# zihang-student/Codes-of-IPD-SsN-AMG-method

Hardware: AMD Instinct MI355X
Metric: V-cycle throughput (DoF*cycles/sec), m=n=1024 OT grid (higher is better)
Workload: dtype f64

## Files before the change

codes_of_ipd_ssn_amg_method_amd/csrc/ipd_resident.h:

```cpp
#pragma once

#include "ipd_resident_proto.h"

static constexpr int RES_P3_LD = 1152;
static constexpr int RES_P4_LD = 2 * RES_P4_SEG + 64;

struct ResLevelDesc {
    int N, nf, S;
    const unsigned short* pci;
    const double* pva;
    const double* diag;
    const double* dinv;
    const double* Axi;
    const double* xx;
};
struct ResDesc {
    ResLevelDesc L1, L2;
    ResLevelDesc L3;
    ResCsr Pt2, P2;
    ResCsr Pt3, P3;
    ResCsr Pt4, P4;
    ResCsr A3;
    ResCsr A4;
    int three;
    const double* p3rows;
    const double* p3w;
    const double* p2rows;
    const double* p2w;
    int p2seg, p2ld;
    int N5;
    const double* p4rows;
    const double* p4w;
    int remote;
    ResTail tail;
    int xm, xm_nwf, xm_nwc;
    const unsigned long long* xm_fbits;
    const unsigned long long* xm_cbits;
    const double* xm_beta;
    const double* xm_rho;
    int localfirst;
    int wident;
    int Nt;
    int nu, isnsp, wcycle, anycycle, maxit;
    double retol;
    long long pcg_maxit;
    unsigned char* gran0;
    unsigned char* gran1;
    int presleep;
    int pollsleep;
    unsigned* tmo;
    long long* dbg;
    unsigned dbg_skip_seq;
};

template <int KE>
// ... 43 lines not shown
    double y[KE];
#pragma unroll
    for (int q = 0; q < KE / 2; ++q) {
        asm volatile("" : "+v"(c[q]));
        const unsigned lo = c[q] & 0xffffu, hi = c[q] >> 16;
        y[2 * q] = *reinterpret_cast<const double*>(smb + OFFB + lo);
        y[2 * q + 1] = *reinterpret_cast<const double*>(smb + OFFB + hi);
    }
    double s0 = a[0] * y[0], s1 = a[1] * y[1], s2 = a[2] * y[2], s3 = a[3] * y[3];
#pragma unroll
    for (int q = 4; q < KE; q += 4) {
        s0 = __builtin_fma(a[q], y[q], s0);
        s1 = __builtin_fma(a[q + 1], y[q + 1], s1);
        s2 = __builtin_fma(a[q + 2], y[q + 2], s2);
        s3 = __builtin_fma(a[q + 3], y[q + 3], s3);
    }
    return (s0 + s1) + (s2 + s3);
}

__device__ __forceinline__ double res_csr_rowdot(const ResCsr& M, int e0, int e1, int lane,
                                                 const double* sm, int off) {
    double s = 0.0;
    for (int t = e0 + lane; t < e1; t += 64 * 8) {
        int jj[8];
        double aa[8];
#pragma unroll
        for (int u = 0; u < 8; ++u) {
            const int tt = t + 64 * u;
            const int tc = tt < e1 ? tt : e0;
            jj[u] = M.ci[tc];
            aa[u] = M.va[tc];
        }
#pragma unroll
        for (int u = 0; u < 8; ++u) s += (t + 64 * u < e1) ? aa[u] * sm[off + jj[u]] : 0.0;
    }
    return wave_sum(s);
}

__device__ __forceinline__ double res_red8(const double* red) {
    double t = 0.0;
#pragma unroll
    for (int k = 0; k < RES_WAVES; ++k) t += red[k];
    return t;
}

__device__ __forceinline__ double res_red8_tree(const double* red) {
    static_assert(RES_WAVES == 8, "eight waves");
    double v[RES_WAVES];
#pragma unroll
    for (int k = 0; k < RES_WAVES; ++k) v[k] = red[k];
    return ((v[0] + v[1]) + (v[2] + v[3])) + ((v[4] + v[5]) + (v[6] + v[7]));
}

__device__ __forceinline__ void res_swap_halves32(double& a, double& b) {
    const auto lo = __builtin_amdgcn_permlane32_swap((unsigned)__double2loint(a), (unsigned)__double2loint(b), false, false);
    const auto hi = __builtin_amdgcn_permlane32_swap((unsigned)__double2hiint(a), (unsigned)__double2hiint(b), false, false);
    a = __hiloint2double((int)hi[0], (int)lo[0]);
    b = __hiloint2double((int)hi[1], (int)lo[1]);
}
__device__ __forceinline__ void res_swap_rows16(double& a, double& b) {
    const auto lo = __builtin_amdgcn_permlane16_swap((unsigned)__double2loint(a), (unsigned)__double2loint(b), false, false);
    const auto hi = __builtin_amdgcn_permlane16_swap((unsigned)__double2hiint(a), (unsigned)__double2hiint(b), false, false);
    a = __hiloint2double((int)hi[0], (int)lo[0]);
    b = __hiloint2double((int)hi[1], (int)lo[1]);
}
__device__ __forceinline__ void res_cs_rows(const double (&A)[RES_WAVES][2], double v0, double v1, double* part_out,
                                            int w, int lane) {
    static_assert(RES_WAVES == 8, "eight rows per block and workgroup");
    double p[RES_WAVES];
#pragma unroll
    for (int r = 0; r < RES_WAVES; ++r) p[r] = __builtin_fma(A[r][1], v1, A[r][0] * v0);
    double q[4];
#pragma unroll
    for (int k = 0; k < 4; ++k) {
        res_swap_halves32(p[k], p[k + 4]);
        q[k] = p[k] + p[k + 4];
    }
    double t[2];
#pragma unroll
    for (int k = 0; k < 2; ++k) {
        res_swap_rows16(q[k], q[k + 2]);
        t[k] = q[k] + q[k + 2];
    }
    const bool f = (lane & 8) != 0;
    const double keep = f ? t[1] : t[0], send = f ? t[0] : t[1];
    double u = keep + dpp_get<0x128, 0xf>(send);
    u = subwave_sum(u, 8);
    if ((lane & 7) == 0) part_out[8 * (lane >> 3) + w] = u;
}

enum res_class {
    RES_CL_HALF = 0,
    RES_CL_START = 1,
    RES_CL_RR = 2,
    RES_CL_RESTRICT = 3,
    RES_CL_LEVEL2 = 4,
    RES_CL_PROLONG = 5,
    RES_CL_TOP = 6,
    RES_NCLASS = 8
};

template <int KE1, int KE2, int KE3 = 0, bool POLY2 = false, bool DIAG = true, bool FULL = false>
__global__ __launch_bounds__(BT, 2) void k_resident(const ResDesc D, const double* __restrict__ bvec,
                                                    double* xg, double* out, int fixed_cycles) {
    static_assert(!POLY2 || (KE3 == 0 && KE1 == 16), "POLY2: three-level hierarchies in column slices (resident_takes_poly2)");
    static_assert(!FULL || POLY2, "FULL: the composed instantiation only (resident_takes_full)");
    static_assert(DIAG || KE1 == 16, "the production form exists for the column-slice kernels");
    constexpr int FG = 2 * BT / RES_WAVES;
    if constexpr (FULL) __builtin_assume(__builtin_amdgcn_workitem_id_x() < (unsigned)BT);
    constexpr bool THREE = KE3 > 0;
    constexpr bool POLY3 = KE3 == 1;
    constexpr int K3 = (THREE && !POLY3) ? KE3 : 2;
    extern __shared__ __attribute__((aligned(16))) char res_smem[];
    double* sm = reinterpret_cast<double*>(res_smem);
    const char* smb = res_smem;
    const int tid = threadIdx.x, w = tid >> 6, lane = tid & 63;
#define RES_REMOTE (FULL ? 0 : D.remote)
#define RES_WIDENT (FULL ? 1 : D.wident)
    const int b = blockIdx.x, G = FULL ? FG : gridDim.x - (RES_REMOTE ? 1 : 0);
    const int N1 = FULL ? 4 * BT : D.L1.N, N2 = FULL ? 2 * BT : D.L2.N, nf = FULL ? 2 * BT : D.L1.nf, nc = N1 - nf;
    const int Nt = FULL ? 1 : D.Nt;
    if (RES_REMOTE && b == G) {
        __shared__ PhaseLds tail_lds;
        __shared__ double tail_red[16];
        __shared__ double tail_part[48 + SOLVE_ML + 1];
        __shared__ int tail_stat[RES_WAVES];
        res_tail_workgroup(D.tail, res_smem, &tail_lds, tail_red, tail_part, tail_stat);
        return;
    }
    constexpr int oX = 0, oE1 = RES_NMAX, oE2 = 2 * RES_NMAX, oRR1 = 3 * RES_NMAX;
    constexpr int oR1 = 4 * RES_NMAX, oAX1 = 5 * RES_NMAX, oR2 = 6 * RES_NMAX, oRR2 = 7 * RES_NMAX;
    constexpr int oAX2 = 8 * RES_NMAX;
    constexpr int oRHO = 9 * RES_NMAX;
    constexpr int oBETA = oAX2 + RES_NMAX / 2;
    constexpr int oU = oRR2;
    constexpr int oR3 = 9 * RES_NMAX + RES_NMAX / 2, oE3 = oR3 + RES_TAIL_MAX, oP3 = oE3 + RES_TAIL_MAX;
    constexpr int oPART = oR3, oPART9 = oR3 + 2 * RES_WAVES * RES_WAVES;
    static_assert(2 * RES_WAVES * RES_WAVES + 2 * RES_WAVES <= 3 * RES_TAIL_MAX, "the totals fit the tail's slots");
    constexpr int oRED = oP3 + RES_TAIL_MAX;
    constexpr int oPUB = oRED + 2 * RES_WAVES;
    constexpr int oOWN = oPUB + 2 * RES_WAVES;
// ... 127 lines not shown
        rowp[12 * w + 2] = D.P2.rp[rF];
        rowp[12 * w + 3] = vF ? D.P2.rp[rF + 1] : D.P2.rp[rF];
        rowp[12 * w + 4] = D.P2.rp[rC];
        rowp[12 * w + 5] = vC ? D.P2.rp[rC + 1] : D.P2.rp[rC];
        const int rin = b + G * w;
        const ResCsr& Pin = D.tail.root == 4 ? D.Pt4 : D.Pt3;
        rowp[12 * w + 6] = (RES_REMOTE && rin < Nt) ? Pin.rp[rin] : 0;
        rowp[12 * w + 7] = (RES_REMOTE && rin < Nt) ? Pin.rp[rin + 1] : 0;
        rowp[12 * w + 8] = v3 ? D.Pt3.rp[r3] : 0;
        rowp[12 * w + 9] = v3 ? D.Pt3.rp[r3 + 1] : 0;
        rowp[12 * w + 10] = (THREE && v2) ? D.P3.rp[r2] : 0;
        rowp[12 * w + 11] = (THREE && v2) ? D.P3.rp[r2 + 1] : 0;
    }
#define dgF sm[oOWN + 0 * RES_WAVES + w]
#define dvF sm[oOWN + 1 * RES_WAVES + w]
#define bF sm[oOWN + 2 * RES_WAVES + w]
#define dgC sm[oOWN + 3 * RES_WAVES + w]
#define dvC sm[oOWN + 4 * RES_WAVES + w]
#define bC sm[oOWN + 5 * RES_WAVES + w]
#define dg2 sm[oOWN + 6 * RES_WAVES + w]
#define dv2 sm[oOWN + 7 * RES_WAVES + w]
#define dg3 sm[oOWN + 8 * RES_WAVES + w]
#define dv3 sm[oOWN + 9 * RES_WAVES + w]
    const bool nsp = FULL ? true : D.isnsp != 0;
    const double xx1 = nsp ? D.L1.xx[0] : 1.0, xx2 = nsp ? D.L2.xx[0] : 1.0;
    const double xx3 = (THREE && nsp) ? D.L3.xx[0] : 1.0;
    const double rxx1 = 1.0 / xx1, rxx2 = 1.0 / xx2, rxx3 = 1.0 / xx3;
    for (int j = tid; j < N1; j += BT) {
        sm[oX + j] = xg[j];
        sm[oE1 + j] = 0.0;
        sm[oAX1 + j] = D.L1.Axi[j];
    }
    for (int j = tid; j < N2; j += BT) {
        sm[oE2 + j] = 0.0;
        sm[oAX2 + j] = D.L2.Axi[j];
    }
    if (THREE)
        for (int j = tid; j < N3; j += BT) {
            sm[oE3L + j] = 0.0;
            sm[oAX3L + j] = D.L3.Axi[j];
        }
    const bool tail1 = FULL ? true : !THREE && Nt == 1 && N2 <= RES_NMAX / 2;
    constexpr int oP3C = oRR2 + RES_NMAX / 2;
    const bool lfirst = FULL ? true : D.localfirst && D.nu >= 1 && N2 <= RES_NMAX / 2 && nf <= RES_NMAX / 2;
    const bool lfirst2 = lfirst && !THREE;
    constexpr int oDV1 = oR2 + RES_NMAX / 2, oDV2 = oE2 + RES_NMAX / 2;
    if (lfirst) {
        for (int j = tid; j < nf; j += BT) sm[oDV1 + j] = D.L1.dinv[j];
        if (lfirst2)
            for (int j = tid; j < N2; j += BT) sm[oDV2 + j] = D.L2.dinv[j];
    }
    const bool xm = FULL ? true : !THREE && D.xm != 0 && nc == N2 && D.wident != 0;
    unsigned xbits = 0;
    if (xm) {
        unsigned long long wf[16], wc[16];
#pragma unroll
        for (int q = 0; q < 16; ++q) {
            wf[q] = D.xm_fbits[(size_t)rF * D.xm_nwf + (q < D.xm_nwf ? q : 0)];
            wc[q] = D.xm_cbits[(size_t)(rC - nf) * D.xm_nwc + (q < D.xm_nwc ? q : 0)];
        }
        unsigned lo = 0, hi = 0;
#pragma unroll
        for (int q = 0; q < 16; ++q) {
            lo |= (vF && q < D.xm_nwf) ? (unsigned)((wf[q] >> lane) & 1ull) << q : 0u;
            hi |= (vC && q < D.xm_nwc) ? (unsigned)((wc[q] >> lane) & 1ull) << q : 0u;
        }
        xbits = lo | (hi << 16);
        for (int j = tid; j < nf; j += BT) sm[oRHO + j] = D.xm_rho[j];
        for (int j = tid; j < nc; j += BT) sm[oBETA + j] = D.xm_beta[j];
    }
    double h33 = 0.0;
    if (tail1) {
        for (int j = tid; j < N2; j += BT) {
            double v = 0.0;
            if (POLY2) {
                v = D.p2rows[(size_t)N2 * D.p2ld + j];
            } else {
                for (int t = D.P3.rp[j]; t < D.P3.rp[j + 1]; ++t)
                    if (D.P3.ci[t] == 0) v = D.P3.va[t];
            }
            sm[oP3C + j] = v;
        }
        for (int t = D.A3.rp[0]; t < D.A3.rp[1]; ++t)
            if (D.A3.ci[t] == 0) h33 = D.A3.va[t];
    }
    if (tid == 0) *fail = 0;
    __syncthreads();

    const auto rs = __builtin_amdgcn_make_buffer_rsrc(D.gran0, 0, 2 * RES_GRAN_MAX * 16, 0x00020000);
    unsigned seq = 0;
    bool dead = false;
    const bool dbg = DIAG && D.dbg != nullptr && b == 0 && tid == 0;
#define RES_SKIPPED(sq) (DIAG && (sq) == D.dbg_skip_seq && b == G - 1)
    if (dbg) {
        dbg_acc[0] = dbg_acc[3] = dbg_acc[4] = dbg_acc[5] = dbg_acc[6] = dbg_acc[7] = dbg_acc[8] = 0;
        dbg_acc[1] = __builtin_amdgcn_s_memtime();
        dbg_acc[2] = __builtin_amdgcn_s_memrealtime();
        if constexpr (KE1 == 16)
            for (int k = 0; k < 2 * RES_NCLASS; ++k) cls_acc[k] = 0u;
    }
    auto cls_begin = [&](int c) __attribute__((always_inline)) {
        if constexpr (KE1 == 16) {
            if (dbg) __hip_atomic_fetch_sub(cls_acc + c, (unsigned)__builtin_amdgcn_s_memtime(), __ATOMIC_RELAXED, __HIP_MEMORY_SCOPE_WORKGROUP);
        }
    };
    auto cls_end = [&](int c) __attribute__((always_inline)) {
// ... 106 lines not shown
    (void)csFed; (void)csBuf; (void)eFo; (void)eCo;
    bool topfed = false;
    (void)topfed;
    auto cs_both_rows = [&](int off) __attribute__((always_inline)) {
        const double f0 = tid < nc ? sm[off + nf + tid] : 0.0, f1 = tid + BT < nc ? sm[off + nf + tid + BT] : 0.0;
        const double g0 = tid < nf ? sm[off + tid] : 0.0, g1 = tid + BT < nf ? sm[off + tid + BT] : 0.0;
        res_cs_rows(AF, f0, f1, sm + oPART, w, lane);
        res_cs_rows(AC, g0, g1, sm + oPART + RES_WAVES * RES_WAVES, w, lane);
        csFed = -1;
        eFo = eCo = 0.0;
    };

    auto cs_row_value = [&](int off, bool rhs_b) __attribute__((always_inline)) {
        const bool sec = lane >= RES_WAVES;
        const int r = lane & (RES_WAVES - 1);
        const int row = sec ? RES_OWN_ROW(loC, hiC, r) : RES_OWN_ROW(loF, hiF, r);
        const double T = res_red8_tree(sm + oPART + RES_WAVES * lane);
        const double dg_ = sm[oOWN + (sec ? 3 : 0) * RES_WAVES + r];
        const double base = rhs_b ? sm[oOWN + (sec ? 5 : 2) * RES_WAVES + r] : sm[oR1 + row];
        return base - (T + dg_ * sm[off + row]);
    };

    auto top = [&]() __attribute__((always_inline)) {
        double nrm2 = 0.0, sumr = 0.0;
        bool fed = false;
        if constexpr (FULL) {
            if (topfed) {
                fed = true;
                topfed = false;
                ++seq;
                if (*fail) dead = true;
                double hv[4];
                if (dbg) dbg_acc[0] -= __builtin_amdgcn_s_memtime();
                for (int ps = 0; ps < D.presleep; ++ps) __builtin_amdgcn_s_sleep(1);
                if (res_sweep<4>(rs, seq, N1, dead, D.tmo, hv, D.pollsleep)) {
                    *fail = 1;
                    if (lane == 0) __hip_atomic_store(D.tmo, seq, __ATOMIC_RELAXED, __HIP_MEMORY_SCOPE_AGENT);
                }
                if (dbg) {
                    const long long t_ = __builtin_amdgcn_s_memtime();
                    dbg_acc[0] += t_;
                    dbg_acc[4] -= t_;
                }
                double p0 = 0.0, p1 = 0.0;
#pragma unroll
                for (int u = 0; u < 4; ++u) {
                    const int j = tid + u * BT;
                    const double v = hv[u];
                    sm[oR1 + j] = v;
                    sm[oE1 + j] = 0.0;
                    p0 += v * v;
                    p1 += v;
                }
                p0 = wave_sum(p0);
                p1 = wave_sum(p1);
                if (lane == 0) {
                    red[w] = p0;
                    red[RES_WAVES + w] = p1;
                }
                if (dbg) {
                    const long long t_ = __builtin_amdgcn_s_memtime();
                    dbg_acc[4] += t_;
                    dbg_acc[5] -= t_;
                }
                __syncthreads();
                if (dbg) dbg_acc[5] += __builtin_amdgcn_s_memtime();
                nrm2 = res_red8_tree(red);
                sumr = res_red8_tree(red + RES_WAVES);
            }
        }
        if (!fed) {
        if constexpr (CS1) {
            cls_begin(RES_CL_TOP);
            cs_both_rows(oX);
        } else {
        const double sF = wave_sum(res_rowdot_fma<KR1, 8 * oX>(cF, aF, smb));
        const double sC = wave_sum(res_rowdot_fma<KR1, 8 * oX>(cC, aC, smb));
        if (lane == 0) {
            sm[oPUB + w] = bF - (sF + dgF * sm[oX + rF]);
            sm[oPUB + RES_WAVES + w] = bC - (sC + dgC * sm[oX + rC]);
        }
        }
        if constexpr (CS1)
            RES_HANDOFF_PV(4, N1, loF, hiF - loF, loC, hiC - loC, cs_row_value(oX, true), {},
                           { sm[oR1 + j] = v; sm[oE1 + j] = 0.0; p0 += v * v; p1 += v; }, {}, 2, nrm2, sumr);
        else
        RES_HANDOFF(4, N1, loF, hiF - loF, loC, hiC - loC,
                    { sm[oR1 + j] = v; sm[oE1 + j] = 0.0; p0 += v * v; p1 += v; }, {}, 2, nrm2, sumr);
        }
        c1 = nsp ? sumr * rxx1 : 0.0;
        if constexpr (FULL) {
            double e0[2];
#pragma unroll
            for (int u = 0; u < 2; ++u) {
                const int j = tid + u * BT;
                const double g_i = sm[oR1 + j] - sm[oAX1 + j] * c1;
                e0[u] = sm[oDV1 + j] * g_i;
                sm[oE1 + j] = e0[u];
            }
            csBuf ^= 1;
            res_cs_rows(AC, e0[0], e0[1], sm + oPART + RES_WAVES * RES_WAVES * csBuf, w, lane);
            {
                const int row = loF + (lane & (RES_WAVES - 1));
                const double g_i = sm[oR1 + row] - sm[oAX1 + row] * c1;
                eFo = sm[oDV1 + row] * g_i;
                eCo = 0.0;
            }
            csFed = 1;
// ... 565 lines not shown
            (void)keep;
        } else if (THREE) {
            const int nu = D.nu;
            for (int s = 0; s < nu; ++s) sweep3(!keep && s == 0);
            {
                const double s = wave_sum(res_rowdot<K3, 8 * oE3L>(c3, a3, smb)) + dg3 * sm[oE3L + r3];
                if (lane == 0) sm[oPUB + w] = sm[oR3L + r3] - s;
                RES_HANDOFF3({ sm[oRR3L + j] = v; }, 0, dum0);
            }
            if (RES_REMOTE)
                remote_tail(D.Pt4, oRR3L, oE3L, oR3L, oAX3L, xx3, N3, c3s);
            else
                local_tail(D.Pt4, D.A4, D.P4, oRR3L, oE3L, oR3L, oAX3L, xx3, N3, c3s);
            for (int s = 0; s < nu; ++s) sweep3(false);
        }
    };

    auto visit2 = [&](bool keep) __attribute__((always_inline)) {
        const int nu = D.nu;
        for (int s = (lfirst2 && !keep) ? 1 : 0; s < nu; ++s) sweep2(!keep && s == 0);
        {
            cls_begin(RES_CL_LEVEL2);
            const double s = wave_sum(res_rowdot_fma<KE2, 8 * oE2>(c2, a2, smb)) + dg2 * sm[oE2 + r2];
            if (lane == 0) sm[oPUB + w] = sm[oR2 + r2] - s;
            RES_HANDOFF(4, N2, lo2, hi2 - lo2, 0, 0, { sm[oRR2 + j] = v; }, {}, 0, dum0, dum1);
        }
        if (dbg) dbg_acc[7] -= __builtin_amdgcn_s_memtime();
        if (THREE) {
            {
                const double s = res_csr_rowdot(D.Pt3, rowp[12 * w + 8], rowp[12 * w + 9], lane, sm, oRR2);
                if (lane == 0) sm[oPUB + w] = s;
                double sumr = 0.0;
                RES_HANDOFF3({ sm[oR3L + j] = v; sm[oE3L + j] = 0.0; p0 += v; }, (nsp ? 1 : 0), sumr);
                c3s = nsp ? sumr * rxx3 : 0.0;
                sumr3 = sumr;
            }
            for (int leg = 0; leg < (D.wcycle ? 2 : 1); ++leg) visit3(leg == 1);
            {
                const double sP = res_csr_rowdot(D.P3, rowp[12 * w + 10], rowp[12 * w + 11], lane, sm, oE3L);
                if (lane == 0) sm[oPUB + w] = sm[oE2 + r2] + sP;
                double xig = 0.0;
                RES_HANDOFF_P(4, N2, lo2, hi2 - lo2, 0, 0, { pa_[u_] = sm[oR2 + j]; pb_[u_] = sm[oAX2 + j]; },
                              { sm[oE2 + j] = v; p0 += pa_[u_] - pb_[u_] * v; }, {}, (nsp ? 1 : 0), xig, dum1);
                c2s = nsp ? xig * rxx2 : 0.0;
            }
        } else {
            tail();
        }
        if (dbg) dbg_acc[7] += __builtin_amdgcn_s_memtime();
        cls_end(RES_CL_LEVEL2);
        for (int s = 0; s < nu; ++s) sweep2(false);
    };

    auto poly2_fed = [&]() __attribute__((always_inline)) {
        if constexpr (POLY2) {
            ++seq;
            if (*fail) dead = true;
            if (dbg) dbg_acc[3] -= __builtin_amdgcn_s_memtime();
            __syncthreads();
            if (dbg) dbg_acc[3] += __builtin_amdgcn_s_memtime();
            const bool pub = w == 0 && lane < RES_WAVES && lane < hi2 - lo2;
            if (pub && !RES_SKIPPED(seq)) res_publish(rs, seq, lo2 + lane, sm[oPUB + lane]);
            const double s0 = tid < N2 ? sm[oP3C + tid] : 0.0, s1 = tid + BT < N2 ? sm[oP3C + tid + BT] : 0.0;
            double hv[2] = {0.0, 0.0};
            if (dbg) dbg_acc[0] -= __builtin_amdgcn_s_memtime();
            for (int ps = 0; ps < D.presleep; ++ps) __builtin_amdgcn_s_sleep(1);
            if (res_sweep<2>(rs, seq, N2, dead, D.tmo, hv, D.pollsleep)) {
                *fail = 1;
                if (lane == 0) __hip_atomic_store(D.tmo, seq, __ATOMIC_RELAXED, __HIP_MEMORY_SCOPE_AGENT);
            }
            if (dbg) {
                const long long t_ = __builtin_amdgcn_s_memtime();
                dbg_acc[0] += t_;
                dbg_acc[4] -= t_;
            }
            const double v0 = tid < N2 ? hv[0] : 0.0, v1 = tid + BT < N2 ? hv[1] : 0.0;
            res_cs_rows(B2, v0, v1, sm + oPART, w, lane);
            const double ps = wave_sum(s0 * v0 + s1 * v1);
            const double p1 = nsp ? wave_sum(v0 + v1) : 0.0;
            if (lane == 0) {
                red[w] = ps;
                red[RES_WAVES + w] = p1;
            }
            if (dbg) {
                const long long t_ = __builtin_amdgcn_s_memtime();
                dbg_acc[4] += t_;
                dbg_acc[3] -= t_;
            }
            __syncthreads();
            if (dbg) dbg_acc[3] += __builtin_amdgcn_s_memtime();
            cls_end(RES_CL_RESTRICT);
            cls_begin(RES_CL_LEVEL2);
            ++seq;
            if (*fail) dead = true;
            if (w == 0 && lane < RES_WAVES) {
                const double wB = sm[oOWN + 6 * RES_WAVES + lane], mp = sm[oOWN + 7 * RES_WAVES + lane];
                const double T = res_red8_tree(sm + oPART + RES_WAVES * lane);
                const double sr = res_red8_tree(red), sum1 = res_red8_tree(red + RES_WAVES);
                const double d = res_pcg_1x1(sr + p2ws * sum1, h33, D.pcg_maxit);
                const double val = T + wB * sum1 + mp * d;
                if (pub && !RES_SKIPPED(seq)) res_publish(rs, seq, lo2 + lane, val);
            }
            double be[2] = {0.0, 0.0};
            (void)be;
            if constexpr (FULL) {
                be[0] = sm[oBETA + tid];
                be[1] = sm[oBETA + tid + BT];
            }
            if (dbg) dbg_acc[0] -= __builtin_amdgcn_s_memtime();
            for (int ps = 0; ps < D.presleep; ++ps) __builtin_amdgcn_s_sleep(1);
            if (res_sweep<2>(rs, seq, N2, dead, D.tmo, hv, D.pollsleep)) {
                *fail = 1;
                if (lane == 0) __hip_atomic_store(D.tmo, seq, __ATOMIC_RELAXED, __HIP_MEMORY_SCOPE_AGENT);
            }
            if (dbg) {
                const long long t_ = __builtin_amdgcn_s_memtime();
                dbg_acc[0] += t_;
                dbg_acc[4] -= t_;
            }
            if (tid < N2) sm[oE2 + tid] = hv[0];
            if (tid + BT < N2) sm[oE2 + tid + BT] = hv[1];
            if constexpr (FULL) {
                sm[oU + tid] = be[0] * hv[0];
                sm[oU + tid + BT] = be[1] * hv[1];
            }
            if (dbg) {
                const long long t_ = __builtin_amdgcn_s_memtime();
                dbg_acc[4] += t_;
                dbg_acc[5] -= t_;
            }
            __syncthreads();
            if (dbg) dbg_acc[5] += __builtin_amdgcn_s_memtime();
            cls_end(RES_CL_LEVEL2);
        }
    };

    auto cycle = [&]() __attribute__((always_inline)) {
        const int nu = D.nu;
        if constexpr (FULL) cs_finish(false, false, false, seq + 1);
        for (int s = 0; s < nu; ++s) sweep1(false, s == 0, s == nu - 1, s == 0);
        if constexpr (FULL) {
            ++seq;
            if (*fail) dead = true;
            const double rh0 = sm[oRHO + tid], rh1 = sm[oRHO + tid + BT];
            double hv[2] = {0.0, 0.0};
            if (dbg) dbg_acc[0] -= __builtin_amdgcn_s_memtime();
            for (int ps = 0; ps < D.presleep; ++ps) __builtin_amdgcn_s_sleep(1);
            if (res_sweep<2>(rs, seq, nf, dead, D.tmo, hv, D.pollsleep)) {
                *fail = 1;
                if (lane == 0) __hip_atomic_store(D.tmo, seq, __ATOMIC_RELAXED, __HIP_MEMORY_SCOPE_AGENT);
            }
            if (dbg) {
                const long long t_ = __builtin_amdgcn_s_memtime();
                dbg_acc[0] += t_;
                dbg_acc[4] -= t_;
            }
            sm[oRR1 + tid] = hv[0] * rh0;
            sm[oRR1 + tid + BT] = hv[1] * rh1;
            if (dbg) {
                const long long t_ = __builtin_amdgcn_s_memtime();
                dbg_acc[4] += t_;
                dbg_acc[5] -= t_;
            }
            __syncthreads();
            if (dbg) dbg_acc[5] += __builtin_amdgcn_s_memtime();
        } else
        {
            if constexpr (CS1) {
                cls_begin(RES_CL_RR);
                cs_both_rows(oE1);
            } else {
            const double sF = wave_sum(res_rowdot_fma<KR1, 8 * oE1>(cF, aF, smb)) + dgF * sm[oE1 + rF];
            const double sC = wave_sum(res_rowdot_fma<KR1, 8 * oE1>(cC, aC, smb)) + dgC * sm[oE1 + rC];
            if (lane == 0) {
                sm[oPUB + w] = sm[oR1 + rF] - sF;
                sm[oPUB + RES_WAVES + w] = sm[oR1 + rC] - sC;
            }
            }
            if constexpr (CS1) {
                if (xm) {
                    RES_HANDOFF_PV(4, N1, loF, hiF - loF, loC, hiC - loC, cs_row_value(oE1, false),
                                   { pa_[u_] = j < nf ? sm[oRHO + j] : 1.0; },
                                   { sm[oRR1 + j] = j < nf ? v * pa_[u_] : v; }, {}, 0, dum0, dum1);
                } else {
                    RES_HANDOFF_PV(4, N1, loF, hiF - loF, loC, hiC - loC, cs_row_value(oE1, false), {},
                                   { sm[oRR1 + j] = v; }, {}, 0, dum0, dum1);
                }
            } else
            if (xm) {
                RES_HANDOFF_P(4, N1, loF, hiF - loF, loC, hiC - loC, { pa_[u_] = j < nf ? sm[oRHO + j] : 1.0; },
                              { sm[oRR1 + j] = j < nf ? v * pa_[u_] : v; }, {}, 0, dum0, dum1);
            } else {
                RES_HANDOFF(4, N1, loF, hiF - loF, loC, hiC - loC, { sm[oRR1 + j] = v; }, {}, 0, dum0, dum1);
            }
        }
        {
            cls_end(RES_CL_RR);
            cls_begin(RES_CL_RESTRICT);
            if (dbg) dbg_acc[6] -= __builtin_amdgcn_s_memtime();
            const double s = xm ? sm[oBETA + r2] * masked_sum(xbits >> 16, oRR1, nf) + sm[oRR1 + rC]
                                : res_csr_rowdot(D.Pt2, rowp[12 * w + 0], rowp[12 * w + 1], lane, sm, oRR1) +
                                      (RES_WIDENT ? sm[oRR1 + rC] : 0.0);
            if (dbg) dbg_acc[6] += __builtin_amdgcn_s_memtime();
            if (lane == 0) sm[oPUB + w] = s;
            if constexpr (POLY2) {
                poly2_fed();
            } else {
            double sumr = 0.0;
            RES_HANDOFF(4, N2, lo2, hi2 - lo2, 0, 0, { sm[oR2 + j] = v; sm[oE2 + j] = 0.0; p0 += v; }, {},
                        (nsp ? 1 : 0), sumr, dum1);
            c2s = nsp ? sumr * rxx2 : 0.0;
            sumr2p = sumr;
            if (lfirst2 && !POLY2) {
                const double cc = c2s;
                double p0 = 0.0;
                for (int j = tid; j < N2; j += BT) {
                    const double g_i = sm[oR2 + j] - sm[oAX2 + j] * cc;
                    const double en = sm[oDV2 + j] * g_i + cc;
                    sm[oE2 + j] = en;
                    p0 += sm[oR2 + j] - sm[oAX2 + j] * en;
                }
                if (nsp) {
                    p0 = wave_sum(p0);
                    if (lane == 0) red[w] = p0;
                }
                __syncthreads();
                if (nsp) c2s = res_red8(red) / xx2;
                __syncthreads();
            }
            cls_end(RES_CL_RESTRICT);
            }
        }
        if constexpr (!POLY2)
            for (int leg = 0; leg < (D.wcycle ? 2 : 1); ++leg) visit2(leg == 1);
        {
            cls_begin(RES_CL_PROLONG);
            if (dbg) dbg_acc[6] -= __builtin_amdgcn_s_memtime();
            if constexpr (FULL) {
                const double sF = sm[oRHO + rF] * masked_sum(xbits & 0xffffu, oU, N2);
                if (dbg) dbg_acc[6] += __builtin_amdgcn_s_memtime();
                if (lane == 0) sm[oPUB + w] = sm[oE1 + rF] + sF;
                ++seq;
                if (*fail) dead = true;
                if (dbg) dbg_acc[3] -= __builtin_amdgcn_s_memtime();
                __syncthreads();
                if (dbg) dbg_acc[3] += __builtin_amdgcn_s_memtime();
                if (w == 0 && lane < RES_WAVES && !RES_SKIPPED(seq)) res_publish(rs, seq, loF + lane, sm[oPUB + lane]);
                double pa[2], pb[2], tc[2], hv[2] = {0.0, 0.0};
#pragma unroll
                for (int u = 0; u < 2; ++u) {
                    const int j = tid + u * BT;
                    pa[u] = sm[oR1 + j];
                    pb[u] = sm[oAX1 + j];
                    const double ec = sm[oE1 + nf + j] + sm[oE2 + j];
                    sm[oE1 + nf + j] = ec;
                    tc[u] = sm[oR1 + nf + j] - sm[oAX1 + nf + j] * ec;
                }
                if (dbg) dbg_acc[0] -= __builtin_amdgcn_s_memtime();
                for (int ps = 0; ps < D.presleep; ++ps) __builtin_amdgcn_s_sleep(1);
                if (res_sweep<2>(rs, seq, nf, dead, D.tmo, hv, D.pollsleep)) {
                    *fail = 1;
                    if (lane == 0) __hip_atomic_store(D.tmo, seq, __ATOMIC_RELAXED, __HIP_MEMORY_SCOPE_AGENT);
                }
                if (dbg) {
                    const long long t_ = __builtin_amdgcn_s_memtime();
                    dbg_acc[0] += t_;
                    dbg_acc[4] -= t_;
                }
                double p0 = 0.0;
#pragma unroll
                for (int u = 0; u < 2; ++u) {
                    sm[oE1 + tid + u * BT] = hv[u];
                    p0 += pa[u] - pb[u] * hv[u];
                }
                p0 += tc[0];
                p0 += tc[1];
                csBuf ^= 1;
                res_cs_rows(AC, hv[0], hv[1], sm + oPART + RES_WAVES * RES_WAVES * csBuf, w, lane);
                p0 = wave_sum(p0);
                if (lane == 0) red[w] = p0;
                if (dbg) {
                    const long long t_ = __builtin_amdgcn_s_memtime();
                    dbg_acc[4] += t_;
                    dbg_acc[5] -= t_;
                }
                __syncthreads();
                if (dbg) dbg_acc[5] += __builtin_amdgcn_s_memtime();
                c1 = res_red8_tree(red) * rxx1;
                eFo = sm[oE1 + loF + (lane & (RES_WAVES - 1))];
                eCo = sm[oE1 + loC + (lane & (RES_WAVES - 1))];
                cs_finish(false, true, false, seq + 1);
                csFed = 1;
                cls_end(RES_CL_PROLONG);
            } else {
            if (xm) {
                for (int j = tid; j < N2; j += BT) sm[oU + j] = sm[oBETA + j] * sm[oE2 + j];
                __syncthreads();
            }
            const double sF = xm ? sm[oRHO + rF] * masked_sum(xbits & 0xffffu, oU, N2)
                                 : res_csr_rowdot(D.P2, rowp[12 * w + 2], rowp[12 * w + 3], lane, sm, oE2);
            const double sC = RES_WIDENT ? sm[oE2 + r2]
                                       : res_csr_rowdot(D.P2, rowp[12 * w + 4], rowp[12 * w + 5], lane, sm, oE2);
            if (dbg) dbg_acc[6] += __builtin_amdgcn_s_memtime();
            if (lane == 0) {
                sm[oPUB + w] = sm[oE1 + rF] + sF;
                sm[oPUB + RES_WAVES + w] = sm[oE1 + rC] + sC;
            }
            double xig = 0.0;
            if constexpr (CS1) {
                const bool fedpost = FULL ? true : nu >= 1 && nf <= 2 * BT;
                double fe[2] = {0.0, 0.0};
                RES_HANDOFF_PVA(4, N1, loF, hiF - loF, loC, hiC - loC, sm[oPUB + lane],
                                { pa_[u_] = sm[oR1 + j]; pb_[u_] = sm[oAX1 + j]; },
                                {
                                    sm[oE1 + j] = v;
                                    p0 += pa_[u_] - pb_[u_] * v;
                                    if (u_ < 2 && j < nf) fe[u_] = v;
                                },
                                {
                                    if (fedpost) {
                                        csBuf ^= 1;
                                        res_cs_rows(AC, fe[0], fe[1], sm + oPART + RES_WAVES * RES_WAVES * csBuf, w, lane);
                                    }
                                },
                                {}, (nsp ? 1 : 0), xig, dum1);
                c1 = nsp ? xig * rxx1 : 0.0;
                if (fedpost) {
                    eFo = sm[oE1 + RES_OWN_ROW(loF, hiF, lane)];
                    eCo = sm[oE1 + RES_OWN_ROW(loC, hiC, lane)];
                    cs_finish(false, true, false, seq + 1);
                    csFed = 1;
                }
                cls_end(RES_CL_PROLONG);
            } else {
            RES_HANDOFF_P(4, N1, loF, hiF - loF, loC, hiC - loC, { pa_[u_] = sm[oR1 + j]; pb_[u_] = sm[oAX1 + j]; },
                          { sm[oE1 + j] = v; p0 += pa_[u_] - pb_[u_] * v; }, {}, (nsp ? 1 : 0), xig, dum1);
            c1 = nsp ? xig * rxx1 : 0.0;
            }
            }
        }
        for (int s = 0; s < nu; ++s) sweep1(true, false, s == nu - 1, s == 0 && csFed != 1);
    };

    auto add_correction = [&]() __attribute__((always_inline)) {
        if constexpr (FULL) {
            if (topfed) return;
        }
        for (int j = tid; j < N1; j += BT) sm[oX + j] = sm[oX + j] + sm[oE1 + j];
        __syncthreads();
    };

    const int maxit = D.maxit;
    const bool writer = b == 0 && tid == 0;
    const ResSolve sol = res_stationary(top, cycle, add_correction, D.retol, maxit, D.anycycle, fixed_cycles, dead, writer, out);
    if (RES_REMOTE && b == 0 && tid == 0)
        __hip_atomic_store(D.tail.tctl, 1u, __ATOMIC_RELAXED, __HIP_MEMORY_SCOPE_AGENT);
    if (b == 0)
        for (int j = tid; j < N1; j += BT) xg[j] = sm[oX + j];
    if (writer) {
        out[0] = (double)sol.it;
        out[1] = sol.rel_res;
        out[2] = sol.res0;
        const unsigned anytmo = __hip_atomic_load(D.tmo, __ATOMIC_ACQUIRE, __HIP_MEMORY_SCOPE_AGENT);
        out[3] = (dead || anytmo != 0) ? 1.0 : 0.0;
        if (CS1 && __hip_atomic_load(D.tmo + 1, __ATOMIC_RELAXED, __HIP_MEMORY_SCOPE_AGENT) != 0) out[3] = 2.0;
        out[4 + 2 * (maxit + 2) - 1] = (double)(seq + tseq);
    }
    if (dbg) {
        D.dbg[0] = dbg_acc[0];
        D.dbg[1] = __builtin_amdgcn_s_memtime() - dbg_acc[1];
        D.dbg[2] = seq;
        D.dbg[3] = __builtin_amdgcn_s_memrealtime() - dbg_acc[2];
        D.dbg[4] = dbg_acc[3];
        D.dbg[5] = dbg_acc[4];
        D.dbg[6] = dbg_acc[5];
        D.dbg[7] = dbg_acc[6];
        D.dbg[8] = dbg_acc[7];
        if (CS1 && !RES_REMOTE) D.dbg[9] = dbg_acc[8];
        if constexpr (CS1)
            for (int k = 0; k < 2 * RES_NCLASS; ++k) D.dbg[16 + k] = (long long)cls_acc[k];
    }
#undef RES_REMOTE
#undef RES_WIDENT
#undef RES_OWN_ROW
#undef RES_SKIPPED
#undef RES_HANDOFF3
#undef RES_HANDOFF3R
#undef RES_HANDOFF4
#undef RES_HANDOFF
#undef RES_HANDOFF_P
#undef RES_HANDOFF_PV
#undef RES_HANDOFF_PVA
#undef dgF
#undef dvF
#undef bF
#undef dgC
#undef dvC
#undef bC
#undef dg2
#undef dv2
#undef dg3
#undef dv3
}
```

codes_of_ipd_ssn_amg_method_amd/csrc/ipd_resident_plan.h:

```cpp
#pragma once

#include <tuple>

#include "ipd_level_plan.h"

enum ResidentKind { RESIDENT_NONE, RESIDENT_K, RESIDENT_BIG, RESIDENT_DEEP };

struct ResidentKey {
    bool big = false;
    int ke = 0, ke3 = 0;
    bool poly2 = false;
    int ke2 = 0, rpw = 0;
    bool deep = false;
    bool full = false;
    static ResidentKey k(int ke, int ke3, bool poly2) { return ResidentKey{false, ke, ke3, poly2, 0, 0, false}; }
    static ResidentKey mask(int ke2, int rpw, bool deep) { return ResidentKey{true, 0, 0, false, ke2, rpw, deep}; }
    bool operator==(const ResidentKey& o) const {
        return std::tie(big, ke, ke3, poly2, ke2, rpw, deep, full) ==
               std::tie(o.big, o.ke, o.ke3, o.poly2, o.ke2, o.rpw, o.deep, o.full);
    }
};

struct ResidentImage {
    bool have = false;
// ... 115 lines not shown
    const int N5r = in.J >= 6 ? in.L[5].nr : 0;
    const bool poly4 = poly3 && in.have5() && N1 <= RES_NMAX && N5r >= 1 && N5r <= 64 && N5r <= G &&
                       N4 <= RES_P4_SEG && N4 + G <= BT;
    size_t tail_lds = remote ? in.img[tail].lds : 0, tail_bm = remote ? in.img[tail].bm : 0;
    if (poly4) {
        tail = in.sub5;
        tail_lds = in.img[tail].lds;
        tail_bm = 0;
    }
    if (!remote || tail_lds + tail_bm > RES_LDS_MAX) tail_bm = 0;
    const size_t lds = remote ? std::max<size_t>(RES_LDS_BYTES, tail_lds + tail_bm) : RES_LDS_BYTES;
    if (lds > RES_LDS_MAX) return p;
    p.kind = RESIDENT_K;
    p.key = ResidentKey::k(ke, ke3, false);
    p.G = G;
    p.lds = lds;
    p.remote = remote;
    p.three = three;
    p.poly3 = poly3;
    p.poly4 = poly4;
    p.tail_root = poly4 ? 5 : three ? 4 : 3;
    p.Nin = Nin;
    p.tail_image = remote ? tail : IMG_NONE;
    p.tail_bm = remote && tail_bm > 0;
    p.priv[3] = three && !poly3 && in.S[3] <= 0;
    p.wident = N2 != nc ? 0 : in.bigph ? 1 : -1;
    p.levels = poly4 ? 4 : ke3 > 0 ? 3 : 2;
    return p;
}

inline bool resident_takes_poly2(const ResidentPlan& p, const ResidentInputs& in) {
    if (p.kind != RESIDENT_K || p.key.poly2 || p.remote || p.key.ke3 != 0 || p.key.ke != 16) return false;
    return in.J == 3 && p.Nin == 1 && !p.three && in.cycle == 'v' && in.smoth >= 1 && in.L[2].nr <= RES_NMAX / 2 &&
           in.L[1].nf <= RES_NMAX / 2 && in.L[2].nr <= 64 * 16;
}

struct ResidentFullFacts {
    bool mask_transfers;
    int wident;
    int isnsp;
    bool localfirst;
};

inline bool resident_takes_full(const ResidentPlan& p, const ResidentInputs& in, const ResidentFullFacts& f,
                                const PlanSwitches& sw) {
    if (sw.res_no_full || p.kind != RESIDENT_K || !p.key.poly2 || p.key.ke != 16 || p.key.ke3 != 0 || p.remote || p.three)
        return false;
    if (in.J != 3 || p.Nin != 1 || in.cycle != 'v' || in.smoth < 1) return false;
    const int nf = in.L[1].nf, nc = in.L[1].nr - nf, N2 = in.L[2].nr;
    if (nf != 2 * BT || nc != 2 * BT || N2 != 2 * BT || p.G * RES_WAVES != nf) return false;
    return f.mask_transfers && f.wident == 1 && f.isnsp == 1 && f.localfirst;
}

inline bool resident_wants_mask_transfers(const ResidentInputs& in, const ResidentFacts& f) {
    return f.ok && f.wident && in.J == 3;
}
inline bool resident_mask_transfers_fit(const ResidentInputs& in, const ResidentFacts& f) {
    return in.L[1].nf <= RES_NMAX / 2 && in.L[2].nr == f.m;
}

inline ResidentPlan plan_resident_big(const ResidentInputs& in, const PlanSwitches& sw, const ResidentFacts& f) {
    ResidentPlan p;
    const int n = f.n, m = f.m;
    const int G = resident_cdiv(std::max(n, m), RES_WAVES);
    if (!(!sw.no_resident && !f.off && !sw.no_resident_big && (sw.resident_big || (!f.ok && n + m > RES_NMAX)) &&
          !in.small_ok && !f.mask_form && in.J == 3 && in.L[3].nr == 1 && n <= RB_HALF && m <= RB_HALF &&
          in.L[2].nr == m && in.cyc() && !in.twogrid && G <= in.num_cu && G <= std::min(n, m) && in.smoth >= 1))
        return p;
    p.S[2] = resident_stride(in, 2, &p.priv[2]);
    if (!(p.S[2] > 0 && p.S[2] <= 64 * 32)) return p;
    p.kind = RESIDENT_BIG;
    p.key = ResidentKey::mask(p.S[2] <= 64 * 16 ? 16 : 32, 1, false);
    p.G = G;
    p.lds = RB_LDS_BYTES;
    p.tail_root = 3;
    p.levels = 2;
    p.ranks = std::max(1, std::min(8, sw.resident_ranks));
    if (p.ranks > G) p.ranks = 1;
    return p;
}

static inline ImageRole resident_deep_image(const ResidentInputs& in) {
    if ((in.k_sub == 4 && in.img[IMG_SUB].have) || (in.k_sub == 5 && in.have5())) return IMG_SUB;
    if (in.k_sub == 3 && in.img[IMG_SUB4].have) return IMG_SUB4;
    return IMG_NONE;
}

inline bool resident_deep_candidate(const ResidentInputs& in, const PlanSwitches& sw, const ResidentFacts& f) {
    const ImageRole img = resident_deep_image(in);
    return !sw.no_resident && !sw.no_resident_big && !sw.no_resident_deep && !f.off && !f.ok && !f.mask_form &&
           !in.small_ok && !in.twogrid && in.cyc() && in.smoth >= 1 && in.J >= 5 &&
           (f.n + f.m > RES_NMAX || sw.resident_big) && in.L[1].nf == f.n && in.L[1].nr == f.m + f.n &&
           resident_deep_sizes_fit(f.n, f.m, in.L[2].nr, in.L[3].nr, in.L[4].nr) && img != IMG_NONE &&
           std::max(RB_LDS_BYTES, in.img[img].lds) <= RES_LDS_MAX;
}

inline ResidentPlan plan_resident_deep(const ResidentInputs& in, const PlanSwitches& sw, const ResidentFacts& f) {
    ResidentPlan p;
    if (!resident_deep_candidate(in, sw, f)) return p;
    const int n = f.n, m = f.m, N3 = in.L[3].nr, N4 = in.L[4].nr;
    int G = std::max(std::max(resident_cdiv(std::max(n, m), 2 * RES_WAVES), resident_cdiv(N3, 4)), std::max(N4, 128));
    G = std::max(G, sw.resident_g);
    p.S[2] = resident_stride(in, 2, &p.priv[2]);
    const int N5 = in.J >= 6 ? in.L[5].nr : 0;
    const bool poly4 = in.have5() && in.k_sub == 5 && N4 <= 2 * G && N5 >= 1 && N5 <= G && N5 <= RB_N5MAX &&
                       N4 + G <= BT && std::max(RB_LDS_BYTES, in.img[in.sub5].lds) <= RES_LDS_MAX;
// ... 15 lines not shown
```

Baseline: 57.75 million.

## Compute masked restriction/prolongation via column-slice butterfly reductions, dropping barriers

Replaces the per-row masked sums over shared vectors in the resident V-cycle's mask-transfer path with column-sliced bit masks, reduced through the cross-lane butterfly into double-buffered partial slots. Restriction and prolongation values are then published directly from the partials. In the FULL path this removes a block barrier and the shared staging of the level-2 correction. It also fuses paired wave reductions into one interleaved DPP sequence. This reorganizes the bit-mask layout and the handoff ordering, which risks stale buffer reads if the csBuf toggling is mis-sequenced.

```diff
diff --git a/codes_of_ipd_ssn_amg_method_amd/csrc/ipd_resident.h b/codes_of_ipd_ssn_amg_method_amd/csrc/ipd_resident.h
--- a/codes_of_ipd_ssn_amg_method_amd/csrc/ipd_resident.h
+++ b/codes_of_ipd_ssn_amg_method_amd/csrc/ipd_resident.h
@@ -1,6 +1,7 @@
 #pragma once
 
 #include "ipd_resident_proto.h"
+#include "ipd_resident_plan.h"
 
 static constexpr int RES_P3_LD = 1152;
 static constexpr int RES_P4_LD = 2 * RES_P4_SEG + 64;
@@ -150,6 +151,27 @@
     return ((v[0] + v[1]) + (v[2] + v[3])) + ((v[4] + v[5]) + (v[6] + v[7]));
 }
 
+__device__ __forceinline__ void wave_sum2(double& a, double& b) {
+#define RES_WS2_STEP(CTRL, MASK)                          \
+    {                                                     \
+        const double ta_ = dpp_get<CTRL, MASK>(a);        \
+        const double tb_ = dpp_get<CTRL, MASK>(b);        \
+        a += ta_;                                         \
+        b += tb_;                                         \
+    }
+    RES_WS2_STEP(0xB1, 0xf)
+    RES_WS2_STEP(0x4E, 0xf)
+    RES_WS2_STEP(0x141, 0xf)
+    RES_WS2_STEP(0x140, 0xf)
+    RES_WS2_STEP(0x142, 0xa)
+    RES_WS2_STEP(0x143, 0xc)
+#undef RES_WS2_STEP
+    const int alo = __builtin_amdgcn_readlane(__double2loint(a), 63), ahi = __builtin_amdgcn_readlane(__double2hiint(a), 63);
+    const int blo = __builtin_amdgcn_readlane(__double2loint(b), 63), bhi = __builtin_amdgcn_readlane(__double2hiint(b), 63);
+    a = __hiloint2double(ahi, alo);
+    b = __hiloint2double(bhi, blo);
+}
+
 __device__ __forceinline__ void res_swap_halves32(double& a, double& b) {
     const auto lo = __builtin_amdgcn_permlane32_swap((unsigned)__double2loint(a), (unsigned)__double2loint(b), false, false);
     const auto hi = __builtin_amdgcn_permlane32_swap((unsigned)__double2hiint(a), (unsigned)__double2hiint(b), false, false);
@@ -162,12 +184,8 @@
     a = __hiloint2double((int)hi[0], (int)lo[0]);
     b = __hiloint2double((int)hi[1], (int)lo[1]);
 }
-__device__ __forceinline__ void res_cs_rows(const double (&A)[RES_WAVES][2], double v0, double v1, double* part_out,
-                                            int w, int lane) {
+__device__ __forceinline__ void res_cs_butterfly(double (&p)[RES_WAVES], double* part_out, int w, int lane) {
     static_assert(RES_WAVES == 8, "eight rows per block and workgroup");
-    double p[RES_WAVES];
-#pragma unroll
-    for (int r = 0; r < RES_WAVES; ++r) p[r] = __builtin_fma(A[r][1], v1, A[r][0] * v0);
     double q[4];
 #pragma unroll
     for (int k = 0; k < 4; ++k) {
@@ -185,6 +203,20 @@
     double u = keep + dpp_get<0x128, 0xf>(send);
     u = subwave_sum(u, 8);
     if ((lane & 7) == 0) part_out[8 * (lane >> 3) + w] = u;
+}
+__device__ __forceinline__ void res_cs_rows(const double (&A)[RES_WAVES][2], double v0, double v1, double* part_out,
+                                            int w, int lane) {
+    double p[RES_WAVES];
+#pragma unroll
+    for (int r = 0; r < RES_WAVES; ++r) p[r] = __builtin_fma(A[r][1], v1, A[r][0] * v0);
+    res_cs_butterfly(p, part_out, w, lane);
+}
+__device__ __forceinline__ void res_cs_mask_rows(unsigned bits, double v0, double v1, double* part_out, int w, int lane) {
+    double p[RES_WAVES];
+#pragma unroll
+    for (int r = 0; r < RES_WAVES; ++r)
+        p[r] = (((bits >> res_xfer_pos(0, r, 0)) & 1u) ? v0 : 0.0) + (((bits >> res_xfer_pos(0, r, 1)) & 1u) ? v1 : 0.0);
+    res_cs_butterfly(p, part_out, w, lane);
 }
 
 enum res_class {
@@ -418,6 +450,38 @@
     }
     const bool xm = FULL ? true : !THREE && D.xm != 0 && nc == N2 && D.wident != 0;
     unsigned xbits = 0;
+    if (CS1 && xm) {
+        const int nwc = FULL ? 2 * BT / 64 : D.xm_nwc, nwf = FULL ? 2 * BT / 64 : D.xm_nwf;
+        const unsigned* cb32 = reinterpret_cast<const unsigned*>(D.xm_cbits);
+        const unsigned* fb32 = reinterpret_cast<const unsigned*>(D.xm_fbits);
+        unsigned wc[RES_WAVES][2], wf[RES_WAVES][2];
+        int tq = tid;
+        asm volatile("" : "+v"(tq));
+        unsigned okc = 0, okf = 0;
+#pragma unroll
+        for (int r = 0; r < RES_WAVES; ++r)
+#pragma unroll
+            for (int u = 0; u < 2; ++u) {
+                const int ic = res_xfer_index(nwc, nf, loC - nf, hiC - loC, tq, r, u);
+                const int jf = res_xfer_index(nwf, nc, loF, hiF - loF, tq, r, u);
+                const unsigned hf = (unsigned)res_xfer_shift(res_xfer_col(tq, u)) >> 5;
+                wc[r][u] = cb32[ic >= 0 ? 2u * (unsigned)ic + hf : 0u];
+                wf[r][u] = fb32[jf >= 0 ? 2u * (unsigned)jf + hf : 0u];
+                okc |= ic >= 0 ? 1u << res_xfer_pos(0, r, u) : 0u;
+                okf |= jf >= 0 ? 1u << res_xfer_pos(0, r, u) : 0u;
+            }
+        unsigned lo = 0, hi = 0;
+#pragma unroll
+        for (int r = 0; r < RES_WAVES; ++r)
+#pragma unroll
+            for (int u = 0; u < 2; ++u) {
+                lo |= res_xfer_place32(wc[r][u], tq, r, u);
+                hi |= res_xfer_place32(wf[r][u], tq, r, u);
+            }
+        xbits = (lo & okc) | ((hi & okf) << 16);
+        for (int j = tid; j < nf; j += BT) sm[oRHO + j] = D.xm_rho[j];
+        for (int j = tid; j < nc; j += BT) sm[oBETA + j] = D.xm_beta[j];
+    } else
     if (xm) {
         unsigned long long wf[16], wc[16];
 #pragma unroll
@@ -630,8 +694,7 @@
                     p0 += v * v;
                     p1 += v;
                 }
-                p0 = wave_sum(p0);
-                p1 = wave_sum(p1);
+                wave_sum2(p0, p1);
                 if (lane == 0) {
                     red[w] = p0;
                     red[RES_WAVES + w] = p1;
@@ -1303,15 +1366,24 @@
         for (int s = 0; s < nu; ++s) sweep2(false);
     };
 
+#define RES_R2_VALUE                                                                                               \
+    ((CS1 && xm) ? sm[oBETA + RES_OWN_ROW(lo2, hi2, lane)] *                                                       \
+                           res_red8_tree(sm + oPART + RES_WAVES * RES_WAVES * csBuf + RES_WAVES * (lane & (RES_WAVES - 1))) + \
+                       sm[oRR1 + RES_OWN_ROW(loC, hiC, lane)]                                                      \
+                 : sm[oPUB + lane])
+    double e2r[2] = {0.0, 0.0};
+    (void)e2r;
     auto poly2_fed = [&]() __attribute__((always_inline)) {
         if constexpr (POLY2) {
             ++seq;
             if (*fail) dead = true;
+            const bool pub = w == 0 && lane < RES_WAVES && lane < hi2 - lo2;
+            if constexpr (!FULL) {
             if (dbg) dbg_acc[3] -= __builtin_amdgcn_s_memtime();
             __syncthreads();
             if (dbg) dbg_acc[3] += __builtin_amdgcn_s_memtime();
-            const bool pub = w == 0 && lane < RES_WAVES && lane < hi2 - lo2;
-            if (pub && !RES_SKIPPED(seq)) res_publish(rs, seq, lo2 + lane, sm[oPUB + lane]);
+            if (pub && !RES_SKIPPED(seq)) res_publish(rs, seq, lo2 + lane, RES_R2_VALUE);
+            }
             const double s0 = tid < N2 ? sm[oP3C + tid] : 0.0, s1 = tid + BT < N2 ? sm[oP3C + tid + BT] : 0.0;
             double hv[2] = {0.0, 0.0};
             if (dbg) dbg_acc[0] -= __builtin_amdgcn_s_memtime();
@@ -1326,9 +1398,15 @@
                 dbg_acc[4] -= t_;
             }
             const double v0 = tid < N2 ? hv[0] : 0.0, v1 = tid + BT < N2 ? hv[1] : 0.0;
-            res_cs_rows(B2, v0, v1, sm + oPART, w, lane);
-            const double ps = wave_sum(s0 * v0 + s1 * v1);
-            const double p1 = nsp ? wave_sum(v0 + v1) : 0.0;
+            csBuf ^= 1;
+            res_cs_rows(B2, v0, v1, sm + oPART + RES_WAVES * RES_WAVES * csBuf, w, lane);
+            double ps = s0 * v0 + s1 * v1, p1 = v0 + v1;
+            if (nsp)
+                wave_sum2(ps, p1);
+            else {
+                ps = wave_sum(ps);
+                p1 = 0.0;
+            }
             if (lane == 0) {
                 red[w] = ps;
                 red[RES_WAVES + w] = p1;
@@ -1346,7 +1424,7 @@
             if (*fail) dead = true;
             if (w == 0 && lane < RES_WAVES) {
                 const double wB = sm[oOWN + 6 * RES_WAVES + lane], mp = sm[oOWN + 7 * RES_WAVES + lane];
-                const double T = res_red8_tree(sm + oPART + RES_WAVES * lane);
+                const double T = res_red8_tree(sm + oPART + RES_WAVES * RES_WAVES * csBuf + RES_WAVES * lane);
                 const double sr = res_red8_tree(red), sum1 = res_red8_tree(red + RES_WAVES);
                 const double d = res_pcg_1x1(sr + p2ws * sum1, h33, D.pcg_maxit);
                 const double val = T + wB * sum1 + mp * d;
@@ -1369,11 +1447,14 @@
                 dbg_acc[0] += t_;
                 dbg_acc[4] -= t_;
             }
+            if constexpr (FULL) {
+                e2r[0] = hv[0];
+                e2r[1] = hv[1];
+                csBuf ^= 1;
+                res_cs_mask_rows(xbits >> 16, be[0] * hv[0], be[1] * hv[1], sm + oPART + RES_WAVES * RES_WAVES * csBuf, w, lane);
+            } else {
             if (tid < N2) sm[oE2 + tid] = hv[0];
             if (tid + BT < N2) sm[oE2 + tid + BT] = hv[1];
-            if constexpr (FULL) {
-                sm[oU + tid] = be[0] * hv[0];
-                sm[oU + tid + BT] = be[1] * hv[1];
             }
             if (dbg) {
                 const long long t_ = __builtin_amdgcn_s_memtime();
@@ -1383,6 +1464,15 @@
             __syncthreads();
             if (dbg) dbg_acc[5] += __builtin_amdgcn_s_memtime();
             cls_end(RES_CL_LEVEL2);
+            if constexpr (FULL) {
+                cls_begin(RES_CL_PROLONG);
+                if (w == 0 && lane < RES_WAVES) {
+                    const double T = res_red8_tree(sm + oPART + RES_WAVES * RES_WAVES * csBuf + RES_WAVES * lane);
+                    const double sF = sm[oRHO + loF + lane] * T;
+                    const double val = sm[oE1 + loF + lane] + sF;
+                    if (!RES_SKIPPED(seq + 1)) res_publish(rs, seq + 1, loF + lane, val);
+                }
+            }
         }
     };
 
@@ -1406,8 +1496,8 @@
                 dbg_acc[0] += t_;
                 dbg_acc[4] -= t_;
             }
-            sm[oRR1 + tid] = hv[0] * rh0;
-            sm[oRR1 + tid + BT] = hv[1] * rh1;
+            csBuf ^= 1;
+            res_cs_mask_rows(xbits & 0xffffu, hv[0] * rh0, hv[1] * rh1, sm + oPART + RES_WAVES * RES_WAVES * csBuf, w, lane);
             if (dbg) {
                 const long long t_ = __builtin_amdgcn_s_memtime();
                 dbg_acc[4] += t_;
@@ -1415,6 +1505,14 @@
             }
             __syncthreads();
             if (dbg) dbg_acc[5] += __builtin_amdgcn_s_memtime();
+            cls_end(RES_CL_RR);
+            cls_begin(RES_CL_RESTRICT);
+            if (w == 0 && lane < RES_WAVES) {
+                const double T = res_red8_tree(sm + oPART + RES_WAVES * RES_WAVES * csBuf + RES_WAVES * lane);
+                const double s = sm[oBETA + lo2 + lane] * T + sm[oRR1 + loC + lane];
+                if (!RES_SKIPPED(seq + 1)) res_publish(rs, seq + 1, lo2 + lane, s);
+            }
+            poly2_fed();
         } else
         {
             if constexpr (CS1) {
@@ -1445,20 +1543,27 @@
                 RES_HANDOFF(4, N1, loF, hiF - loF, loC, hiC - loC, { sm[oRR1 + j] = v; }, {}, 0, dum0, dum1);
             }
         }
-        {
+        if constexpr (!FULL) {
             cls_end(RES_CL_RR);
             cls_begin(RES_CL_RESTRICT);
             if (dbg) dbg_acc[6] -= __builtin_amdgcn_s_memtime();
-            const double s = xm ? sm[oBETA + r2] * masked_sum(xbits >> 16, oRR1, nf) + sm[oRR1 + rC]
+            double s = 0.0;
+            if (CS1 && xm) {
+                const double v0 = tid < nf ? sm[oRR1 + tid] : 0.0, v1 = tid + BT < nf ? sm[oRR1 + tid + BT] : 0.0;
+                csBuf ^= 1;
+                res_cs_mask_rows(xbits & 0xffffu, v0, v1, sm + oPART + RES_WAVES * RES_WAVES * csBuf, w, lane);
+            } else {
+            s = xm ? sm[oBETA + r2] * masked_sum(xbits >> 16, oRR1, nf) + sm[oRR1 + rC]
                                 : res_csr_rowdot(D.Pt2, rowp[12 * w + 0], rowp[12 * w + 1], lane, sm, oRR1) +
                                       (RES_WIDENT ? sm[oRR1 + rC] : 0.0);
+            }
             if (dbg) dbg_acc[6] += __builtin_amdgcn_s_memtime();
             if (lane == 0) sm[oPUB + w] = s;
             if constexpr (POLY2) {
                 poly2_fed();
             } else {
             double sumr = 0.0;
-            RES_HANDOFF(4, N2, lo2, hi2 - lo2, 0, 0, { sm[oR2 + j] = v; sm[oE2 + j] = 0.0; p0 += v; }, {},
+            RES_HANDOFF_PV(4, N2, lo2, hi2 - lo2, 0, 0, RES_R2_VALUE, {}, { sm[oR2 + j] = v; sm[oE2 + j] = 0.0; p0 += v; }, {},
                         (nsp ? 1 : 0), sumr, dum1);
             c2s = nsp ? sumr * rxx2 : 0.0;
             sumr2p = sumr;
@@ -1485,25 +1590,19 @@
         if constexpr (!POLY2)
             for (int leg = 0; leg < (D.wcycle ? 2 : 1); ++leg) visit2(leg == 1);
         {
-            cls_begin(RES_CL_PROLONG);
+            if constexpr (!FULL) cls_begin(RES_CL_PROLONG);
             if (dbg) dbg_acc[6] -= __builtin_amdgcn_s_memtime();
             if constexpr (FULL) {
-                const double sF = sm[oRHO + rF] * masked_sum(xbits & 0xffffu, oU, N2);
                 if (dbg) dbg_acc[6] += __builtin_amdgcn_s_memtime();
-                if (lane == 0) sm[oPUB + w] = sm[oE1 + rF] + sF;
                 ++seq;
                 if (*fail) dead = true;
-                if (dbg) dbg_acc[3] -= __builtin_amdgcn_s_memtime();
-                __syncthreads();
-                if (dbg) dbg_acc[3] += __builtin_amdgcn_s_memtime();
-                if (w == 0 && lane < RES_WAVES && !RES_SKIPPED(seq)) res_publish(rs, seq, loF + lane, sm[oPUB + lane]);
                 double pa[2], pb[2], tc[2], hv[2] = {0.0, 0.0};
 #pragma unroll
                 for (int u = 0; u < 2; ++u) {
                     const int j = tid + u * BT;
                     pa[u] = sm[oR1 + j];
                     pb[u] = sm[oAX1 + j];
-                    const double ec = sm[oE1 + nf + j] + sm[oE2 + j];
+                    const double ec = sm[oE1 + nf + j] + e2r[u];
                     sm[oE1 + nf + j] = ec;
                     tc[u] = sm[oR1 + nf + j] - sm[oAX1 + nf + j] * ec;
                 }
@@ -1544,12 +1643,22 @@
                 csFed = 1;
                 cls_end(RES_CL_PROLONG);
             } else {
+            double sF = 0.0;
+            if (CS1 && xm) {
+                const double v0 = tid < N2 ? sm[oBETA + tid] * sm[oE2 + tid] : 0.0;
+                const double v1 = tid + BT < N2 ? sm[oBETA + tid + BT] * sm[oE2 + tid + BT] : 0.0;
+                csBuf ^= 1;
+                res_cs_mask_rows(xbits >> 16, v0, v1, sm + oPART + RES_WAVES * RES_WAVES * csBuf, w, lane);
+                __syncthreads();
+                sF = sm[oRHO + rF] * res_red8_tree(sm + oPART + RES_WAVES * RES_WAVES * csBuf + RES_WAVES * w);
+            } else {
             if (xm) {
                 for (int j = tid; j < N2; j += BT) sm[oU + j] = sm[oBETA + j] * sm[oE2 + j];
                 __syncthreads();
             }
-            const double sF = xm ? sm[oRHO + rF] * masked_sum(xbits & 0xffffu, oU, N2)
+            sF = xm ? sm[oRHO + rF] * masked_sum(xbits & 0xffffu, oU, N2)
                                  : res_csr_rowdot(D.P2, rowp[12 * w + 2], rowp[12 * w + 3], lane, sm, oE2);
+            }
             const double sC = RES_WIDENT ? sm[oE2 + r2]
                                        : res_csr_rowdot(D.P2, rowp[12 * w + 4], rowp[12 * w + 5], lane, sm, oE2);
             if (dbg) dbg_acc[6] += __builtin_amdgcn_s_memtime();
@@ -1635,6 +1744,7 @@
 #undef RES_WIDENT
 #undef RES_OWN_ROW
 #undef RES_SKIPPED
+#undef RES_R2_VALUE
 #undef RES_HANDOFF3
 #undef RES_HANDOFF3R
 #undef RES_HANDOFF4
diff --git a/codes_of_ipd_ssn_amg_method_amd/csrc/ipd_resident_plan.h b/codes_of_ipd_ssn_amg_method_amd/csrc/ipd_resident_plan.h
--- a/codes_of_ipd_ssn_amg_method_amd/csrc/ipd_resident_plan.h
+++ b/codes_of_ipd_ssn_amg_method_amd/csrc/ipd_resident_plan.h
@@ -191,6 +191,37 @@
     return f.mask_transfers && f.wident == 1 && f.isnsp == 1 && f.localfirst;
 }
 
+#define RES_XFER_FN __attribute__((always_inline)) constexpr
+RES_XFER_FN int res_xfer_col(int t, int u) { return t + u * BT; }
+RES_XFER_FN int res_xfer_word(int col) { return col >> 6; }
+RES_XFER_FN int res_xfer_shift(int col) { return col & 63; }
+RES_XFER_FN int res_xfer_pos(int blk, int r, int u) { return 16 * blk + 2 * r + u; }
+RES_XFER_FN int res_xfer_index(int nw, int ncol, int row0, int cnt, int t, int r, int u) {
+    const int col = res_xfer_col(t, u);
+    return (r < cnt && col < ncol && res_xfer_word(col) < nw) ? (row0 + r) * nw + res_xfer_word(col) : -1;
+}
+RES_XFER_FN unsigned res_xfer_place32(unsigned half, int t, int r, int u) {
+    return ((half >> (res_xfer_shift(res_xfer_col(t, u)) & 31)) & 1u) << res_xfer_pos(0, r, u);
+}
+RES_XFER_FN unsigned res_xfer_place(unsigned long long wd, int t, int r, int u) {
+    return res_xfer_place32((unsigned)(wd >> (res_xfer_shift(res_xfer_col(t, u)) & 32)), t, r, u);
+}
+RES_XFER_FN unsigned res_xfer_half(const unsigned long long* bits, int nw, int ncol, int row0, int cnt, int t) {
+    unsigned h = 0;
+    for (int r = 0; r < RES_WAVES; ++r)
+        for (int u = 0; u < 2; ++u) {
+            const int i = res_xfer_index(nw, ncol, row0, cnt, t, r, u);
+            if (i >= 0) h |= res_xfer_place(bits[i], t, r, u);
+        }
+    return h;
+}
+RES_XFER_FN unsigned res_xfer_slice_bits(const unsigned long long* cbits, int nwc, int nf, int c0, int cntC,
+                                       const unsigned long long* fbits, int nwf, int nc, int f0, int cntF, int t) {
+    return res_xfer_half(cbits, nwc, nf, c0, cntC, t) | (res_xfer_half(fbits, nwf, nc, f0, cntF, t) << 16);
+}
+
+#undef RES_XFER_FN
+
 inline bool resident_wants_mask_transfers(const ResidentInputs& in, const ResidentFacts& f) {
     return f.ok && f.wident && in.J == 3;
 }
```

Result: no change. 57.93 million (median of 5 runs) (+0.3%).
